# kvas7andy/unreal

Hardware: AMD Instinct MI355X
Metric: env-steps/sec (whole node), UNREAL maze 84x84 (higher is better)
Workload: dtype f32 (fp16x2-split MFMA operands, fp32 accumulate)

## Files before the change

unreal_amd/csrc/gemm_split.hip:

```cpp
#include "common.h"

namespace {

constexpr int BK = 32;
constexpr int NPL = 2;
typedef _Float16 f16x8 __attribute__((ext_vector_type(8)));
typedef _Float16 f16x2 __attribute__((ext_vector_type(2)));
constexpr int ROW_B = 80;
constexpr int FLAG_RELU = 1, FLAG_ACCUM = 2, FLAG_ATOMIC = 4, FLAG_RELU_MASK = 8, FLAG_RELU_BITS = 16;

typedef float f32x2 __attribute__((ext_vector_type(2)));
typedef unsigned int u32x2 __attribute__((ext_vector_type(2)));
typedef unsigned int u32x4 __attribute__((ext_vector_type(4)));

__device__ __forceinline__ int row_deal(int j) { return (j & ~7) | ((j & 1) << 2) | ((j >> 1) & 3); }

struct SplitArgs {
  int M, N, K;
  const float* A; int lda;
  const unsigned short* W; int ldw; long plane;
  float* C; int ldc;
  const float* bias;
  const float* mask; int ldm;
  int flags;
  int vecA;
  int nbx, nby;
  int splitk, ktiles_per_split;
  long slab_stride;
  const float* c_prev; float* c_out; float* h_out; int ld_h;
  const float* A2; int lda2, K1, K1pad;
  const float* dh_above; float* dc_io; const float* gates_act; const float* c_new; float* dpre;
  const float* a_absmax; float a_floor; const float* w_absmax; float* c_absmax0; float* c_absmax1;
};

template <int ROWS, bool VEC>
__device__ __forceinline__ f32x4 a_piece_load(const float* __restrict__ P, int ld, int rows_total, int K, int r0, int k0, int p,
                                              int tid) {
  const int id = tid + 256 * p;
  const int r = min(r0 + row_deal(id / (BK / 4)), rows_total - 1);
  const int k = k0 + (id % (BK / 4)) * 4;
  const float* row = P + (size_t)r * ld;
  if (VEC) return *reinterpret_cast<const f32x4*>(row + min(k, ld - 4));
  f32x4 v;
#pragma unroll
  for (int e = 0; e < 4; ++e) v[e] = row[min(k + e, K - 1)];
  return v;
}

__device__ __forceinline__ void split4_terms(float x0, float x1, float x2, float x3, u32x2 (&pl)[NPL]) {
  const f16x2 h01 = __builtin_convertvector((f32x2){x0, x1}, f16x2), h23 = __builtin_convertvector((f32x2){x2, x3}, f16x2);
  const f32x2 r01 = (f32x2){x0, x1} - __builtin_convertvector(h01, f32x2), r23 = (f32x2){x2, x3} - __builtin_convertvector(h23, f32x2);
  const f16x2 l01 = __builtin_convertvector(r01, f16x2), l23 = __builtin_convertvector(r23, f16x2);
  pl[0] = (u32x2){__builtin_bit_cast(unsigned int, h01), __builtin_bit_cast(unsigned int, h23)};
  pl[1] = (u32x2){__builtin_bit_cast(unsigned int, l01), __builtin_bit_cast(unsigned int, l23)};
}

template <int ROWS>
__device__ __forceinline__ void a_piece_store(unsigned char* S, f32x4 v, int klim, int p, int tid, float scale) {
  const int id = tid + 256 * p;
  const int r = row_deal(id / (BK / 4)), k = (id % (BK / 4)) * 4;
#pragma unroll
  for (int e = 0; e < 4; ++e) v[e] = k + e < klim ? v[e] * scale : 0.f;
  u32x2 pl[NPL];
  split4_terms(v[0], v[1], v[2], v[3], pl);
#pragma unroll
  for (int t = 0; t < NPL; ++t)
    *reinterpret_cast<u32x2*>(S + (t * ROWS + r) * ROW_B + k * 2) = pl[t];
}

template <int ROWS>
__device__ __forceinline__ u32x4 w_piece_load(const unsigned short* __restrict__ W, int ldw, long plane, int rows_total,
                                              int r0, int k0, int p, int tid) {
  const int id = tid + 256 * p;
  const int t = id / (ROWS * 4), r = row_deal((id / 4) % ROWS), c = id % 4;
  const int row = min(r0 + r, rows_total - 1);
  return *reinterpret_cast<const u32x4*>(W + t * plane + (size_t)row * ldw + k0 + c * 8);
}

template <int ROWS>
__device__ __forceinline__ void w_piece_store(unsigned char* S, u32x4 v, int p, int tid) {
  const int id = tid + 256 * p;
  const int t = id / (ROWS * 4), r = row_deal((id / 4) % ROWS), c = id % 4;
  *reinterpret_cast<u32x4*>(S + (t * ROWS + r) * ROW_B + c * 16) = v;
}

template <int BM, int BN, bool SWZ = false>
__device__ __forceinline__ void read_frags(const unsigned char* As, const unsigned char* Bs, int wm, int wn, int li, int kh,
                                           int ks, f16x8 (&af)[BM / 64][NPL], f16x8 (&bf)[BN / 64][NPL]) {
  const int c = 2 * ks + kh;
#pragma unroll
  for (int i = 0; i < BM / 64; ++i)
#pragma unroll
    for (int t = 0; t < NPL; ++t) {
      const int r = wm * (BM / 2) + i * 32 + li;
      af[i][t] = *reinterpret_cast<const f16x8*>(As + (t * BM + r) * ROW_B + (SWZ ? (c ^ ((r >> 4) & 3)) : c) * 16);
    }
#pragma unroll
  for (int j = 0; j < BN / 64; ++j)
#pragma unroll
    for (int t = 0; t < NPL; ++t) {
      const int r = wn * (BN / 2) + j * 32 + li;
      bf[j][t] = *reinterpret_cast<const f16x8*>(Bs + (t * BN + r) * ROW_B + (SWZ ? (c ^ ((r >> 4) & 3)) : c) * 16);
    }
}

template <int TM, int TN>
__device__ __forceinline__ void mma_frags(const f16x8 (&af)[TM][NPL], const f16x8 (&bf)[TN][NPL], f32x16 (&acc)[TM][TN]) {
#pragma unroll
  for (int i = 0; i < TM; ++i)
#pragma unroll
    for (int j = 0; j < TN; ++j) {
      f32x16 c = acc[i][j];
      c = __builtin_amdgcn_mfma_f32_32x32x16_f16(af[i][1], bf[j][0], c, 0, 0, 0);
      c = __builtin_amdgcn_mfma_f32_32x32x16_f16(af[i][0], bf[j][1], c, 0, 0, 0);
      c = __builtin_amdgcn_mfma_f32_32x32x16_f16(af[i][0], bf[j][0], c, 0, 0, 0);
      acc[i][j] = c;
    }
}

template <bool DUAL>
struct ASrc { const float* P; int ld, K, k0; };

template <bool DUAL>
__device__ __forceinline__ ASrc<DUAL> a_src(const SplitArgs& p, int kg) {
  ASrc<DUAL> s;
  if (DUAL) {
    const bool second = kg >= p.K1pad;
    s.P = second ? p.A2 : p.A; s.ld = second ? p.lda2 : p.lda;
    s.K = second ? p.K - p.K1pad : p.K1; s.k0 = second ? kg - p.K1pad : kg;
  } else {
    s.P = p.A; s.ld = p.lda; s.K = p.K; s.k0 = kg;
  }
  return s;
}

template <int BM, int BN, bool VEC, int EPI = 0, int KW = 1, bool DUAL = false>
__global__ __launch_bounds__(256 * KW, KW == 1 ? ((BM == 128 && EPI == 0) ? 3 : 2) : 1) void gemm_split_nt_kernel(SplitArgs p) {
  constexpr bool DEEP = BM == 64;
  constexpr int TM = BM / 64, TN = BN / 64;
  constexpr int PA = BM * BK / 1024, PW = NPL * BN / 64;
  constexpr int A_BYTES = NPL * BM * ROW_B, B_BYTES = NPL * BN * ROW_B;
  const float SA = pow2_scale(fmaxf(p.a_absmax ? *p.a_absmax : 0.f, p.a_floor));
  const float INV_A = pow2_inv(SA);
  const float INV_W = pow2_inv(pow2_scale(*p.w_absmax));
  constexpr bool HALF = BM == 128 && EPI == 0 && KW == 1;
  constexpr int C_BYTES = (HALF ? BM / 2 : BM) * (BN + 4) * 4;
  constexpr int OP_BYTES = A_BYTES + B_BYTES;
  constexpr int RED_BYTES = 64;
  constexpr int SMEM = OP_BYTES > (C_BYTES + RED_BYTES) ? OP_BYTES : (C_BYTES + RED_BYTES);
  static_assert(4 * KW * 4 <= RED_BYTES, "one float per wave");
  __shared__ __attribute__((aligned(16))) unsigned char smem_all[KW * SMEM];
  const int tid = KW == 1 ? (int)threadIdx.x : (int)(threadIdx.x & 255);
  const int grp = KW == 1 ? 0 : (int)(threadIdx.x >> 8);
  unsigned char* smem = smem_all + grp * SMEM;
  unsigned char* As = smem;
  unsigned char* Bs = smem + A_BYTES;

  const int L = blockIdx.x, xcd = L & 7, s = L >> 3;
  const int slab = s % p.splitk, s2 = s / p.splitk;
  const int bx = s2 % p.nbx, by = (s2 / p.nbx) * 8 + xcd;
  if (by >= p.nby) return;
  const int m0 = by * BM, n0 = bx * BN;
  if (EPI == 0) p.C += (size_t)slab * p.slab_stride;
  const int kt_base = slab * p.ktiles_per_split;
  const int nkt = min((p.K + BK - 1) / BK - kt_base, p.ktiles_per_split);
  if (nkt <= 0) return;
  const int lane = tid & 63, wave = tid >> 6;
  const int wm = wave >> 1, wn = wave & 1;
  const int li = lane & 31, kh = lane >> 5;

  f32x16 acc[TM][TN];
#pragma unroll
  for (int i = 0; i < TM; ++i)
#pragma unroll
    for (int j = 0; j < TN; ++j)
#pragma unroll
      for (int r = 0; r < 16; ++r) acc[i][j][r] = 0.f;

  f32x4 ra[2][PA];
  u32x4 rw[PW];
  const int shift = (int)((unsigned)by * 7u % (unsigned)nkt);
#define KT_AT(i) (kt_base + (((i) + shift) >= nkt ? (i) + shift - nkt : (i) + shift))
#define KG_AT(i) (KT_AT(min((i) * KW + grp, nkt - 1)) * BK)
#define KLIM(i, src) ((KW == 1 || (i) * KW + grp < nkt) ? (src).K - (src).k0 : 0)
#define A_LOAD(src, q) a_piece_load<BM, VEC>((src).P, (src).ld, p.M, (src).K, m0, (src).k0, q, tid)
  const int nit = (nkt + KW - 1) / KW;
  {
    const int k0 = KG_AT(0);
    const ASrc<DUAL> s0 = a_src<DUAL>(p, k0);
#pragma unroll
    for (int q = 0; q < PA; ++q) ra[0][q] = A_LOAD(s0, q);
#pragma unroll
    for (int q = 0; q < PW; ++q) rw[q] = w_piece_load<BN>(p.W, p.ldw, p.plane, p.N, n0, k0, q, tid);
#pragma unroll
    for (int q = 0; q < PA; ++q) a_piece_store<BM>(As, ra[0][q], KLIM(0, s0), q, tid, SA);
#pragma unroll
    for (int q = 0; q < PW; ++q) w_piece_store<BN>(Bs, rw[q], q, tid);
    const int k1 = KG_AT(1), k2 = KG_AT(2);
    const ASrc<DUAL> s1 = a_src<DUAL>(p, k1), s2_ = a_src<DUAL>(p, k2);
#pragma unroll
    for (int q = 0; q < PA; ++q) ra[0][q] = A_LOAD(s1, q);
    if (DEEP) {
#pragma unroll
      for (int q = 0; q < PA; ++q) ra[1][q] = A_LOAD(s2_, q);
    }
#pragma unroll
    for (int q = 0; q < PW; ++q) rw[q] = w_piece_load<BN>(p.W, p.ldw, p.plane, p.N, n0, k1, q, tid);
  }
  __syncthreads();

#define SPLIT_NT_TILE(S, IT)                                                                                        \
  {                                                                                                                 \
    f16x8 af[TM][NPL], bf[TN][NPL];                                                                                 \
    read_frags<BM, BN>(As, Bs, wm, wn, li, kh, 0, af, bf);                                                          \
    mma_frags<TM, TN>(af, bf, acc);                                                                                 \
    read_frags<BM, BN>(As, Bs, wm, wn, li, kh, 1, af, bf);          \
    __syncthreads();                                                               \
    const int kcur = KG_AT((IT) + 1), kw = KG_AT((IT) + 2), ka = KG_AT((IT) + (DEEP ? 3 : 2));                      \
    const ASrc<DUAL> scur = a_src<DUAL>(p, kcur), snext = a_src<DUAL>(p, ka);                                       \
    const int klim = KLIM((IT) + 1, scur);                                                                          \
    _Pragma("unroll") for (int q = 0; q < PA; ++q) {                                                                \
      a_piece_store<BM>(As, ra[S][q], klim, q, tid, SA);                                                            \
      ra[S][q] = A_LOAD(snext, q);                                                                                  \
    }                                                                                                               \
    _Pragma("unroll") for (int q = 0; q < PW; ++q) {                                                                \
      w_piece_store<BN>(Bs, rw[q], q, tid);                                                                         \
      rw[q] = w_piece_load<BN>(p.W, p.ldw, p.plane, p.N, n0, kw, q, tid);                                           \
    }                                                                                                               \
    mma_frags<TM, TN>(af, bf, acc);                                                                                 \
    __syncthreads();                                                                    \
  }
  if (DEEP) {
    for (int it = 0; it < nit; it += 2) {
      SPLIT_NT_TILE(0, it)
      if (it + 1 < nit) SPLIT_NT_TILE(1, it + 1)
    }
  } else {
    for (int it = 0; it < nit; ++it) SPLIT_NT_TILE(0, it)
  }
#undef SPLIT_NT_TILE
#undef A_LOAD
#undef KLIM
#undef KG_AT
#undef KT_AT

  if (EPI == 0 && (p.flags & FLAG_ATOMIC)) {
#pragma unroll
    for (int i = 0; i < TM; ++i)
#pragma unroll
      for (int j = 0; j < TN; ++j) {
        const int col = n0 + wn * (BN / 2) + j * 32 + li;
        if (col >= p.N) continue;
        const float bv = (p.bias && slab == 0 && grp == 0) ? p.bias[col] : 0.f;
#pragma unroll
        for (int r = 0; r < 16; ++r) {
          const int row = m0 + wm * (BM / 2) + i * 32 + (r & 3) + 8 * (r >> 2) + 4 * kh;
          const float v = (acc[i][j][r] * INV_A) * INV_W;
          if (row < p.M) atomicAdd(p.C + (size_t)row * p.ldc + col, v + bv);
        }
      }
    return;
  }
  constexpr int CLD = BN + 4;
  float* Cs = reinterpret_cast<float*>(smem);
  if (HALF) {
    const uint16_t* mbits = reinterpret_cast<const uint16_t*>(p.mask);
    const bool vecC = ((p.ldc & 3) == 0) && ((((uintptr_t)p.C) & 15) == 0) &&
                      (!p.bias || ((((uintptr_t)p.bias) & 15) == 0)) &&
                      (!(p.flags & FLAG_RELU_MASK) || (((p.ldm & 3) == 0) && ((((uintptr_t)p.mask) & 15) == 0)));
    constexpr int CV = BN / 4;
    float omax = 0.f;
#pragma unroll 1
    for (int half = 0; half < 2; ++half) {
      if (half) __syncthreads();
      if (wm == half) {
#pragma unroll
        for (int i = 0; i < TM; ++i)
#pragma unroll
          for (int j = 0; j < TN; ++j)
#pragma unroll
            for (int r = 0; r < 16; ++r)
              Cs[(i * 32 + (r & 3) + 8 * (r >> 2) + 4 * kh) * CLD + wn * (BN / 2) + j * 32 + li] =
                  (acc[i][j][r] * INV_A) * INV_W;
      }
      __syncthreads();
      for (int id = threadIdx.x; id < (BM / 2) * CV; id += 256) {
        const int r = id / CV, c4 = (id % CV) * 4;
        const int row = m0 + half * (BM / 2) + r, col = n0 + c4;
        if (row >= p.M || col >= p.N) continue;
        f32x4 v = *reinterpret_cast<const f32x4*>(Cs + r * CLD + c4);
        float* cp = p.C + (size_t)row * p.ldc + col;
        if (vecC && col + 3 < p.N) {
          if (p.bias) { const f32x4 b4 = *reinterpret_cast<const f32x4*>(p.bias + col); v += b4; }
          if (p.flags & FLAG_ACCUM) v += *reinterpret_cast<const f32x4*>(cp);
          if (p.flags & FLAG_RELU) {
#pragma unroll
            for (int e = 0; e < 4; ++e) v[e] = fmaxf(v[e], 0.f);
          }
          if (p.flags & FLAG_RELU_MASK) {
            const f32x4 m4 = *reinterpret_cast<const f32x4*>(p.mask + (size_t)row * p.ldm + col);
#pragma unroll
            for (int e = 0; e < 4; ++e) v[e] = m4[e] > 0.f ? v[e] : 0.f;
          }
          if (p.flags & FLAG_RELU_BITS) {
            const unsigned w = mbits[(size_t)row * p.ldm + (col >> 4)] >> (col & 15);
#pragma unroll
            for (int e = 0; e < 4; ++e) v[e] = ((w >> e) & 1u) ? v[e] : 0.f;
          }
          *reinterpret_cast<f32x4*>(cp) = v;
          omax = fmaxf(fmaxf(omax, fmaxf(fabsf(v[0]), fabsf(v[1]))), fmaxf(fabsf(v[2]), fabsf(v[3])));
        } else {
#pragma unroll
          for (int e = 0; e < 4; ++e) {
            if (col + e >= p.N) break;
            float x = v[e] + (p.bias ? p.bias[col + e] : 0.f);
            if (p.flags & FLAG_ACCUM) x += cp[e];
            if (p.flags & FLAG_RELU) x = fmaxf(x, 0.f);
            if (p.flags & FLAG_RELU_MASK) x = (p.mask[(size_t)row * p.ldm + col + e] > 0.f) ? x : 0.f;
            if (p.flags & FLAG_RELU_BITS) x = ((mbits[(size_t)row * p.ldm + ((col + e) >> 4)] >> ((col + e) & 15)) & 1u) ? x : 0.f;
            cp[e] = x;
            omax = fmaxf(omax, fabsf(x));
          }
        }
      }
    }
    if (p.c_absmax0) {
      __syncthreads();
      float* wmx0 = reinterpret_cast<float*>(smem_all);
      omax = wave_max(omax);
      if ((threadIdx.x & 63) == 0) wmx0[threadIdx.x >> 6] = omax;
      __syncthreads();
      if (threadIdx.x < 64) absmax_commit(p.c_absmax0, fmaxf(fmaxf(wmx0[0], wmx0[1]), fmaxf(wmx0[2], wmx0[3])));
    }
    return;
  }
#pragma unroll
  for (int i = 0; i < TM; ++i)
#pragma unroll
    for (int j = 0; j < TN; ++j)
#pragma unroll
      for (int r = 0; r < 16; ++r)
        Cs[(wm * (BM / 2) + i * 32 + (r & 3) + 8 * (r >> 2) + 4 * kh) * CLD + wn * (BN / 2) + j * 32 + li] =
            (acc[i][j][r] * INV_A) * INV_W;
  __syncthreads();
  const float* C0 = reinterpret_cast<const float*>(smem_all);
  constexpr int GSTRIDE = SMEM / 4;
  if (EPI == 1) {
    const int u0 = bx * (BN / 4);
    const bool add_pre = (p.flags & FLAG_ACCUM) != 0;
    constexpr int ITEMS = BM * (BN / 4) / (256 * KW);
    float cprev[ITEMS], pre4[ITEMS][4];
#pragma unroll
    for (int e = 0; e < ITEMS; ++e) {
      const int id = threadIdx.x + e * 256 * KW;
      const int row = min(m0 + id / (BN / 4), p.M - 1), u = u0 + id % (BN / 4);
      cprev[e] = p.c_prev[(size_t)row * 256 + u];
#pragma unroll
      for (int g4 = 0; g4 < 4; ++g4) pre4[e][g4] = add_pre ? p.C[(size_t)row * p.ldc + g4 * 256 + u] : 0.f;
    }
    static_assert((256 * KW) % (BN / 4) == 0, "a lane keeps its hidden unit over the pairs it handles");
    float bb[4];
#pragma unroll
    for (int g4 = 0; g4 < 4; ++g4) bb[g4] = p.bias[g4 * 256 + u0 + threadIdx.x % (BN / 4)];
#pragma unroll
    for (int e = 0; e < ITEMS; ++e) {
      const int id = threadIdx.x + e * 256 * KW;
      const int r = id / (BN / 4), ul = id % (BN / 4);
      const int row = m0 + r, u = u0 + ul;
      const float* cs = C0 + r * CLD + (ul >> 4) * 64 + (ul & 15);
      float s4[4];
#pragma unroll
      for (int g4 = 0; g4 < 4; ++g4) {
        float a = cs[g4 * 16];
#pragma unroll
        for (int g = 1; g < KW; ++g) a += cs[g * GSTRIDE + g4 * 16];
        s4[g4] = add_pre ? a + pre4[e][g4] : a;
      }
      const float gi = 1.f / (1.f + expf(-(s4[0] + bb[0])));
      const float gj = tanhf(s4[1] + bb[1]);
      const float gf = 1.f / (1.f + expf(-(s4[2] + bb[2] + 1.0f)));
      const float go = 1.f / (1.f + expf(-(s4[3] + bb[3])));
      const float c = cprev[e] * gf + gi * gj;
      if (row >= p.M) continue;
      float* pre = p.C + (size_t)row * p.ldc;
      pre[u] = gi; pre[256 + u] = gj; pre[512 + u] = gf; pre[768 + u] = go;
      p.c_out[(size_t)row * 256 + u] = c;
      p.h_out[(size_t)row * p.ld_h + u] = tanhf(c) * go;
    }
    return;
  }
  if (EPI == 2) {
    constexpr int ITEMS = BM * BN / (256 * KW), CH = ITEMS < 4 ? ITEMS : 4;
    float omax = 0.f;
#pragma unroll
    for (int e0 = 0; e0 < ITEMS; e0 += CH) {
      float dha[CH], dcv[CH], cn[CH], cp[CH], ga[CH][4];
#pragma unroll
      for (int e = 0; e < CH; ++e) {
        const int id = threadIdx.x + (e0 + e) * 256 * KW;
        const size_t g = (size_t)min(m0 + id / BN, p.M - 1) * 256 + n0 + id % BN;
        dha[e] = p.dh_above[g]; dcv[e] = p.dc_io[g]; cn[e] = p.c_new[g]; cp[e] = p.c_prev[g];
#pragma unroll
        for (int g4 = 0; g4 < 4; ++g4) ga[e][g4] = p.gates_act[(g / 256) * 1024 + g4 * 256 + g % 256];
      }
#pragma unroll
      for (int e = 0; e < CH; ++e) {
        const int id = threadIdx.x + (e0 + e) * 256 * KW;
        const int r = id / BN, cidx = id % BN;
        float rec = C0[r * CLD + cidx];
#pragma unroll
        for (int g = 1; g < KW; ++g) rec += C0[g * GSTRIDE + r * CLD + cidx];
        if (m0 + r >= p.M) continue;
        const size_t g = (size_t)(m0 + r) * 256 + n0 + cidx;
        const float i = ga[e][0], j = ga[e][1], f = ga[e][2], o = ga[e][3];
        const float dh = dha[e] + rec;
        const float tc = tanhf(cn[e]);
        const float dc = dcv[e] + dh * o * (1.f - tc * tc);
        float* d = p.dpre + (g / 256) * 1024 + g % 256;
        const float d0 = dc * j * i * (1.f - i), d1 = dc * i * (1.f - j * j), d2 = dc * cp[e] * f * (1.f - f),
                    d3 = dh * tc * o * (1.f - o);
        d[0] = d0; d[256] = d1; d[512] = d2; d[768] = d3;
        omax = fmaxf(fmaxf(omax, fmaxf(fabsf(d0), fabsf(d1))), fmaxf(fabsf(d2), fabsf(d3)));
        p.dc_io[g] = dc * f;
      }
    }
    {
      float* wmx = reinterpret_cast<float*>(smem_all + C_BYTES);
      omax = wave_max(omax);
      if ((threadIdx.x & 63) == 0) wmx[threadIdx.x >> 6] = omax;
      __syncthreads();
      if (threadIdx.x < 64) {
        float m = wmx[0];
#pragma unroll
        for (int g = 1; g < 4 * KW; ++g) m = fmaxf(m, wmx[g]);
        absmax_commit(p.c_absmax0, m);
        absmax_commit(p.c_absmax1, m);
      }
    }
    return;
  }
  const uint16_t* mbits = reinterpret_cast<const uint16_t*>(p.mask);
  const bool vecC = ((p.ldc & 3) == 0) && ((((uintptr_t)p.C) & 15) == 0) &&
                    (!p.bias || ((((uintptr_t)p.bias) & 15) == 0)) &&
                    (!(p.flags & FLAG_RELU_MASK) || (((p.ldm & 3) == 0) && ((((uintptr_t)p.mask) & 15) == 0)));
  constexpr int CV = BN / 4;
  float omax = 0.f;
  static_assert((BM * CV) % (256 * KW) == 0, "every lane makes the same number of passes (absmax_commit needs whole waves)");
  for (int id = threadIdx.x; id < BM * CV; id += 256 * KW) {
    const int r = id / CV, c4 = (id % CV) * 4;
    const int row = m0 + r, col = n0 + c4;
    if (row >= p.M || col >= p.N) continue;
    f32x4 v = *reinterpret_cast<const f32x4*>(C0 + r * CLD + c4);
#pragma unroll
    for (int g = 1; g < KW; ++g) v += *reinterpret_cast<const f32x4*>(C0 + g * GSTRIDE + r * CLD + c4);
    float* cp = p.C + (size_t)row * p.ldc + col;
    if (vecC && col + 3 < p.N) {
      if (p.bias) { const f32x4 b4 = *reinterpret_cast<const f32x4*>(p.bias + col); v += b4; }
      if (p.flags & FLAG_ACCUM) v += *reinterpret_cast<const f32x4*>(cp);
      if (p.flags & FLAG_RELU) {
#pragma unroll
        for (int e = 0; e < 4; ++e) v[e] = fmaxf(v[e], 0.f);
      }
      if (p.flags & FLAG_RELU_MASK) {
        const f32x4 m4 = *reinterpret_cast<const f32x4*>(p.mask + (size_t)row * p.ldm + col);
#pragma unroll
        for (int e = 0; e < 4; ++e) v[e] = m4[e] > 0.f ? v[e] : 0.f;
      }
      if (p.flags & FLAG_RELU_BITS) {
        const unsigned w = mbits[(size_t)row * p.ldm + (col >> 4)] >> (col & 15);
#pragma unroll
        for (int e = 0; e < 4; ++e) v[e] = ((w >> e) & 1u) ? v[e] : 0.f;
      }
      *reinterpret_cast<f32x4*>(cp) = v;
      omax = fmaxf(fmaxf(omax, fmaxf(fabsf(v[0]), fabsf(v[1]))), fmaxf(fabsf(v[2]), fabsf(v[3])));
    } else {
#pragma unroll
      for (int e = 0; e < 4; ++e) {
        if (col + e >= p.N) break;
        float x = v[e] + (p.bias ? p.bias[col + e] : 0.f);
        if (p.flags & FLAG_ACCUM) x += cp[e];
        if (p.flags & FLAG_RELU) x = fmaxf(x, 0.f);
        if (p.flags & FLAG_RELU_MASK) x = (p.mask[(size_t)row * p.ldm + col + e] > 0.f) ? x : 0.f;
        if (p.flags & FLAG_RELU_BITS) x = ((mbits[(size_t)row * p.ldm + ((col + e) >> 4)] >> ((col + e) & 15)) & 1u) ? x : 0.f;
        cp[e] = x;
        omax = fmaxf(omax, fabsf(x));
      }
    }
  }
  if (p.c_absmax0) {
    float* wmx0 = reinterpret_cast<float*>(smem_all + C_BYTES);
    omax = wave_max(omax);
    if ((threadIdx.x & 63) == 0) wmx0[threadIdx.x >> 6] = omax;
    __syncthreads();
    if (threadIdx.x < 64) {
      float m = wmx0[0];
#pragma unroll
      for (int g = 1; g < 4 * KW; ++g) m = fmaxf(m, wmx0[g]);
      absmax_commit(p.c_absmax0, m);
    }
  }
}

struct SplitTnArgs {
  int M, N, K;
  const float* A; int lda;
  const float* B; int ldb;
  float* C; int ldc;
  float* colsum;
  int ntx, nty, splitk, ktiles_per_split;
  const float* a_absmax; const float* b_absmax;
};

__device__ __forceinline__ int tn_m4() {
  const int t = threadIdx.x;
  return ((t >> 1) & 1) | (((t >> 4) & 1) << 1) | (((t >> 2) & 3) << 2) | (((t >> 5) & 1) << 4);
}
__device__ __forceinline__ int tn_k4() {
  const int t = threadIdx.x;
  return (t & 1) | ((t >> 6) << 1);
}

__device__ __forceinline__ void tn_piece_load(const float* __restrict__ P, int ld, int K, int c0, int k0, f32x4 (&reg)[4]) {
  const int m4 = tn_m4(), k4 = tn_k4();
  const int col = min(c0 + 4 * m4, ld - 4);
#pragma unroll
  for (int kk = 0; kk < 4; ++kk) {
    const int k = min(k0 + 4 * k4 + kk, K - 1);
    reg[kk] = *reinterpret_cast<const f32x4*>(P + (size_t)k * ld + col);
  }
}

template <int ROWS, bool RAGGED>
__device__ __forceinline__ void tn_piece_store(unsigned char* S, const f32x4 (&reg)[4], int klim, float scale) {
  const int m4 = tn_m4(), k4 = tn_k4();
  bool ok[4];
#pragma unroll
  for (int kk = 0; kk < 4; ++kk) ok[kk] = !RAGGED || 4 * k4 + kk < klim;
#pragma unroll
  for (int j = 0; j < 4; ++j) {
    const int r = 4 * m4 + j;
    u32x2 pl[NPL];
    split4_terms(ok[0] ? reg[0][j] * scale : 0.f, ok[1] ? reg[1][j] * scale : 0.f, ok[2] ? reg[2][j] * scale : 0.f,
                 ok[3] ? reg[3][j] * scale : 0.f, pl);
    const int off = (((k4 >> 1) ^ ((r >> 4) & 3)) * 2 + (k4 & 1)) * 8;
#pragma unroll
    for (int t = 0; t < NPL; ++t)
      *reinterpret_cast<u32x2*>(S + (t * ROWS + r) * ROW_B + off) = pl[t];
  }
}

template <bool RAGGED>
__device__ __forceinline__ void tn_colsum_acc(const f32x4 (&reg)[4], int klim, float w, float (&cs)[4]) {
  const int k4 = tn_k4();
#pragma unroll
  for (int kk = 0; kk < 4; ++kk) {
    const float wk = (!RAGGED || 4 * k4 + kk < klim) ? w : 0.f;
#pragma unroll
    for (int j = 0; j < 4; ++j) cs[j] = fmaf(wk, reg[kk][j], cs[j]);
  }
}

template <bool RAGGED>
__global__ __launch_bounds__(256, 2) void gemm_split_tn_kernel(SplitTnArgs p) {
  constexpr int BM = 128, BN = 128, TM = 2, TN = 2;
  constexpr int A_BYTES = NPL * BM * ROW_B, B_BYTES = NPL * BN * ROW_B;
  constexpr int OP_BYTES = A_BYTES + B_BYTES;
  __shared__ __attribute__((aligned(16))) unsigned char smem[OP_BYTES > 8 * BN * 4 ? OP_BYTES : 8 * BN * 4];
  const float SA = pow2_scale(*p.a_absmax), SB = pow2_scale(*p.b_absmax);
  const float INV_A = pow2_inv(SA), INV_B = pow2_inv(SB);
  unsigned char* As = smem;
  unsigned char* Bs = smem + A_BYTES;

  const int L = blockIdx.x, xcd = L & 7, s = L >> 3;
  const int tiles = p.ntx * p.nty;
  const int slab = (s / tiles) * 8 + xcd, tile = s % tiles;
  if (slab >= p.splitk) return;
  const int bx = tile % p.ntx, by = tile / p.ntx;
  const int m0 = by * BM, n0 = bx * BN;
  const int nk_total = (p.K + BK - 1) / BK;
  const int kt0 = slab * p.ktiles_per_split, kt1 = min(nk_total, kt0 + p.ktiles_per_split);
  if (kt0 >= kt1) return;
  const int nkt = kt1 - kt0;
  const int lane = threadIdx.x & 63, wave = threadIdx.x >> 6;
  const int wm = wave >> 1, wn = wave & 1;
  const int li = lane & 31, kh = lane >> 5;

  f32x16 acc[TM][TN];
#pragma unroll
  for (int i = 0; i < TM; ++i)
#pragma unroll
    for (int j = 0; j < TN; ++j)
#pragma unroll
      for (int r = 0; r < 16; ++r) acc[i][j][r] = 0.f;

  constexpr int TN_FLUSH = 8;
  f32x16 tot[TM][TN];
#pragma unroll
  for (int i = 0; i < TM; ++i)
#pragma unroll
    for (int j = 0; j < TN; ++j)
#pragma unroll
      for (int r = 0; r < 16; ++r) tot[i][j][r] = 0.f;
  f32x4 ra[4], rb[4];
  const float csw = (p.colsum != nullptr && by == 0) ? 1.f : 0.f;
  float cs[4] = {0.f, 0.f, 0.f, 0.f};
  tn_piece_load(p.A, p.lda, p.K, m0, kt0 * BK, ra);
  tn_piece_load(p.B, p.ldb, p.K, n0, kt0 * BK, rb);
  tn_piece_store<BM, RAGGED>(As, ra, p.K - kt0 * BK, SA);
  tn_piece_store<BN, RAGGED>(Bs, rb, p.K - kt0 * BK, SB);
  tn_colsum_acc<RAGGED>(rb, p.K - kt0 * BK, csw, cs);
  {
    const int k1 = (kt0 + min(1, nkt - 1)) * BK;
    tn_piece_load(p.A, p.lda, p.K, m0, k1, ra);
    tn_piece_load(p.B, p.ldb, p.K, n0, k1, rb);
  }
  __syncthreads();

  for (int it = 0; it < nkt; ++it) {
    f16x8 af[TM][NPL], bf[TN][NPL];
    read_frags<BM, BN, true>(As, Bs, wm, wn, li, kh, 0, af, bf);
    mma_frags<TM, TN>(af, bf, acc);
    read_frags<BM, BN, true>(As, Bs, wm, wn, li, kh, 1, af, bf);
    __syncthreads();
    const int kcur = (kt0 + min(it + 1, nkt - 1)) * BK, knext = (kt0 + min(it + 2, nkt - 1)) * BK;
    tn_piece_store<BM, RAGGED>(As, ra, p.K - kcur, SA);
    tn_piece_load(p.A, p.lda, p.K, m0, knext, ra);
    tn_piece_store<BN, RAGGED>(Bs, rb, p.K - kcur, SB);
    tn_colsum_acc<RAGGED>(rb, p.K - kcur, (it + 1 < nkt) ? csw : 0.f, cs);
    tn_piece_load(p.B, p.ldb, p.K, n0, knext, rb);
    mma_frags<TM, TN>(af, bf, acc);
    if ((it + 1) % TN_FLUSH == 0) {
#pragma unroll
      for (int i = 0; i < TM; ++i)
#pragma unroll
        for (int j = 0; j < TN; ++j)
#pragma unroll
          for (int r = 0; r < 16; ++r) { tot[i][j][r] += acc[i][j][r]; acc[i][j][r] = 0.f; }
    }
    __syncthreads();
  }
#pragma unroll
  for (int i = 0; i < TM; ++i)
#pragma unroll
    for (int j = 0; j < TN; ++j)
#pragma unroll
      for (int r = 0; r < 16; ++r) acc[i][j][r] += tot[i][j][r];

  if (csw != 0.f) {
    float* red = reinterpret_cast<float*>(smem);
    const int m4 = tn_m4(), k4 = tn_k4();
#pragma unroll
    for (int j = 0; j < 4; ++j) red[k4 * BN + 4 * m4 + j] = cs[j];
    __syncthreads();
    if (threadIdx.x < BN && n0 + threadIdx.x < p.N) {
      float v = 0.f;
#pragma unroll
      for (int k = 0; k < 8; ++k) v += red[k * BN + threadIdx.x];
      atomicAdd(p.colsum + n0 + threadIdx.x, v);
    }
  }
#pragma unroll
  for (int i = 0; i < TM; ++i)
#pragma unroll
    for (int j = 0; j < TN; ++j) {
      const int col = n0 + wn * (BN / 2) + j * 32 + li;
      if (col >= p.N) continue;
#pragma unroll
      for (int r = 0; r < 16; ++r) {
        const int row = m0 + wm * (BM / 2) + i * 32 + (r & 3) + 8 * (r >> 2) + 4 * kh;
        if (row < p.M) atomicAdd(p.C + (size_t)row * p.ldc + col, (acc[i][j][r] * INV_A) * INV_B);
      }
    }
}

__global__ __launch_bounds__(256) void split_planes_f16x2_kernel(int rows, int cols, const float* __restrict__ src, int ld_src,
                                                                 int transpose, unsigned short* __restrict__ dst, int ld_dst,
                                                                 long plane, int row_perm, const float* __restrict__ w_absmax) {
  __shared__ float t[32][33];
  const float sw = pow2_scale(*w_absmax);
  const int c0 = blockIdx.x * 32, r0 = blockIdx.y * 32;
  const int tx = threadIdx.x & 31, ty = threadIdx.x >> 5;
  for (int y = ty; y < 32; y += 8)
    if (r0 + y < rows && c0 + tx < cols) t[y][tx] = src[(size_t)(r0 + y) * ld_src + c0 + tx];
  __syncthreads();
  for (int y = ty; y < 32; y += 8) {
    int orow = transpose ? c0 + y : r0 + y;
    const int ocol = transpose ? r0 + tx : c0 + tx;
    if (row_perm == 1) orow = ((orow & 255) >> 4) * 64 + (orow >> 8) * 16 + (orow & 15);
    const bool ok = transpose ? (c0 + y < cols && r0 + tx < rows) : (r0 + y < rows && c0 + tx < cols);
    if (!ok) continue;
    const float x = (transpose ? t[tx][y] : t[y][tx]) * sw;
    const _Float16 h = (_Float16)x;
    const _Float16 l = (_Float16)(x - (float)h);
    dst[(size_t)orow * ld_dst + ocol] = __builtin_bit_cast(unsigned short, h);
    dst[plane + (size_t)orow * ld_dst + ocol] = __builtin_bit_cast(unsigned short, l);
  }
}

__global__ __launch_bounds__(256) void absmax_kernel(int rows, int cols, const float* __restrict__ x, int ld, float* slot) {
  float m = 0.f;
  if (ld == cols && (cols & 3) == 0 && ((((uintptr_t)x) & 15) == 0)) {
    const long n4 = (long)rows * cols / 4;
    const f32x4* x4 = reinterpret_cast<const f32x4*>(x);
    for (long i = (long)blockIdx.x * 256 + threadIdx.x; i < n4; i += (long)gridDim.x * 256) {
      const f32x4 v = x4[i];
      m = fmaxf(fmaxf(m, fmaxf(fabsf(v[0]), fabsf(v[1]))), fmaxf(fabsf(v[2]), fabsf(v[3])));
    }
  } else {
    const int wave = (blockIdx.x * 256 + threadIdx.x) >> 6, nw = (gridDim.x * 256) >> 6, lane = threadIdx.x & 63;
    for (int r = wave; r < rows; r += nw)
      for (int c = lane; c < cols; c += 64) m = fmaxf(m, fabsf(x[(size_t)r * ld + c]));
  }
  __shared__ float wm[4];
  m = wave_max(m);
  if ((threadIdx.x & 63) == 0) wm[threadIdx.x >> 6] = m;
  __syncthreads();
  if (threadIdx.x < 64) absmax_commit(slot, fmaxf(fmaxf(wm[0], wm[1]), fmaxf(wm[2], wm[3])));
}

struct MultiAbsDesc { const float* src; float* wmax; long n; long block0; };
struct MultiSplitDesc { const float* src; unsigned short* dst; const float* wmax; long rows, cols, ld_src, transpose, row_perm, ld_dst, plane, tiles_x, block0; };

__global__ __launch_bounds__(256) void multi_absmax_kernel(const MultiAbsDesc* __restrict__ descs, int n_desc) {
// ... 338 lines not shown
```

Before: 3.715 million.

## Peel final K iterations and prefetch LSTM epilogue inputs during last MMA

Peels the last one to two K-loop iterations of the split-fp16 GEMM so the final tiles skip redundant global loads. The global loads for the LSTM forward and backward epilogues (c_prev, previous pre-activations, bias, dh, dc, gate activations) are issued during the last tile's MMA instead of after the loop. This is meant to hide epilogue load latency behind compute. In exchange it raises register pressure, adds complex per-group trip-count logic with extra barrier matching, and pins the FMA contraction in the backward gate math by hand.

```diff
diff --git a/unreal_amd/csrc/gemm_split.hip b/unreal_amd/csrc/gemm_split.hip
--- a/unreal_amd/csrc/gemm_split.hip
+++ b/unreal_amd/csrc/gemm_split.hip
@@ -209,6 +209,39 @@
   }
   __syncthreads();
 
+  constexpr int E1_ITEMS = BM * (BN / 4) / (256 * KW);
+  constexpr int E2_ITEMS = BM * BN / (256 * KW), E2_CH = E2_ITEMS < 4 ? E2_ITEMS : 4;
+  float e1_cprev[E1_ITEMS], e1_pre[E1_ITEMS][4], e1_bias[4];
+  constexpr int E2_PF = E2_CH < 3 ? E2_CH : 3;
+  float e2_in[E2_PF][8];
+  auto epi_prefetch = [&]() __attribute__((always_inline)) {
+    if (EPI == 1) {
+      const int u0 = bx * (BN / 4);
+      const bool add_pre = !DUAL && (p.flags & FLAG_ACCUM) != 0;
+#pragma unroll
+      for (int e = 0; e < E1_ITEMS; ++e) {
+        const int id = threadIdx.x + e * 256 * KW;
+        const int row = min(m0 + id / (BN / 4), p.M - 1), u = u0 + id % (BN / 4);
+        e1_cprev[e] = p.c_prev[(size_t)row * 256 + u];
+#pragma unroll
+        for (int g4 = 0; g4 < 4; ++g4) e1_pre[e][g4] = add_pre ? p.C[(size_t)row * p.ldc + g4 * 256 + u] : 0.f;
+      }
+#pragma unroll
+      for (int g4 = 0; g4 < 4; ++g4) e1_bias[g4] = p.bias[g4 * 256 + u0 + threadIdx.x % (BN / 4)];
+    }
+    if (EPI == 2) {
+#pragma unroll
+      for (int e = 0; e < E2_PF; ++e) {
+        const int id = threadIdx.x + e * 256 * KW;
+        const size_t g = (size_t)min(m0 + id / BN, p.M - 1) * 256 + n0 + id % BN;
+        e2_in[e][0] = p.dh_above[g]; e2_in[e][1] = p.dc_io[g]; e2_in[e][2] = p.c_new[g]; e2_in[e][3] = p.c_prev[g];
+#pragma unroll
+        for (int g4 = 0; g4 < 4; ++g4) e2_in[e][4 + g4] = p.gates_act[(g / 256) * 1024 + g4 * 256 + g % 256];
+      }
+    }
+  };
+  constexpr bool PEEL = !(BM == 128 && EPI == 0);
+
 #define SPLIT_NT_TILE(S, IT)                                                                                        \
   {                                                                                                                 \
     f16x8 af[TM][NPL], bf[TN][NPL];                                                                                 \
@@ -230,14 +263,64 @@
     mma_frags<TM, TN>(af, bf, acc);                                                                                 \
     __syncthreads();                                                                    \
   }
-  if (DEEP) {
-    for (int it = 0; it < nit; it += 2) {
-      SPLIT_NT_TILE(0, it)
-      if (it + 1 < nit) SPLIT_NT_TILE(1, it + 1)
-    }
+#define SPLIT_NT_TAIL(IT, LOAD_W, MID)                                                                              \
+  {                                                                                                                 \
+    f16x8 af[TM][NPL], bf[TN][NPL];                                                                                 \
+    read_frags<BM, BN>(As, Bs, wm, wn, li, kh, 0, af, bf);                                                          \
+    mma_frags<TM, TN>(af, bf, acc);                                                                                 \
+    read_frags<BM, BN>(As, Bs, wm, wn, li, kh, 1, af, bf);                                                          \
+    __syncthreads();                                                                                                \
+    const int kcur = KG_AT((IT) + 1), kw = KG_AT((IT) + 2);                                                         \
+    const ASrc<DUAL> scur = a_src<DUAL>(p, kcur);                                                                   \
+    const int klim = KLIM((IT) + 1, scur);                                                                          \
+    const bool odd = DEEP && (((IT) & 1) != 0);                                                                     \
+    _Pragma("unroll") for (int q = 0; q < PA; ++q) {                                                                \
+      const f32x4 v0 = ra[0][q], v1 = DEEP ? ra[1][q] : v0;                                                         \
+      a_piece_store<BM>(As, odd ? v1 : v0, klim, q, tid, SA);                                                       \
+    }                                                                                                               \
+    _Pragma("unroll") for (int q = 0; q < PW; ++q) {                                                                \
+      w_piece_store<BN>(Bs, rw[q], q, tid);                                                                         \
+      if (LOAD_W) rw[q] = w_piece_load<BN>(p.W, p.ldw, p.plane, p.N, n0, kw, q, tid);                               \
+    }                                                                                                               \
+    MID                                                                                                             \
+    mma_frags<TM, TN>(af, bf, acc);                                                                                 \
+    __syncthreads();                                                                                                \
+  }
+  if (PEEL) {
+    const int nit_g = KW == 1 ? nit : max((nkt - grp + KW - 1) / KW, 1);
+    const int nmain = nit_g - (DEEP ? 3 : 2);
+    if (DEEP) {
+      for (int it = 0; it < nmain; it += 2) {
+        SPLIT_NT_TILE(0, it)
+        if (it + 1 < nmain) SPLIT_NT_TILE(1, it + 1)
+      }
+      if (nit_g >= 3) SPLIT_NT_TAIL(nit_g - 3, true, )
+    } else {
+      for (int it = 0; it < nmain; ++it) SPLIT_NT_TILE(0, it)
+    }
+    if (nit_g >= 2) SPLIT_NT_TAIL(nit_g - 2, false, epi_prefetch();)
+    else epi_prefetch();
+    {
+      f16x8 af[TM][NPL], bf[TN][NPL];
+      read_frags<BM, BN>(As, Bs, wm, wn, li, kh, 0, af, bf);
+      mma_frags<TM, TN>(af, bf, acc);
+      read_frags<BM, BN>(As, Bs, wm, wn, li, kh, 1, af, bf);
+      mma_frags<TM, TN>(af, bf, acc);
+      __syncthreads();
+    }
+    if (KW > 1 && nit_g < nit) { __syncthreads(); __syncthreads(); }
   } else {
-    for (int it = 0; it < nit; ++it) SPLIT_NT_TILE(0, it)
-  }
+    if (DEEP) {
+      for (int it = 0; it < nit; it += 2) {
+        SPLIT_NT_TILE(0, it)
+        if (it + 1 < nit) SPLIT_NT_TILE(1, it + 1)
+      }
+    } else {
+      for (int it = 0; it < nit; ++it) SPLIT_NT_TILE(0, it)
+    }
+    epi_prefetch();
+  }
+#undef SPLIT_NT_TAIL
 #undef SPLIT_NT_TILE
 #undef A_LOAD
 #undef KLIM
@@ -349,19 +432,11 @@
     const int u0 = bx * (BN / 4);
     const bool add_pre = (p.flags & FLAG_ACCUM) != 0;
     constexpr int ITEMS = BM * (BN / 4) / (256 * KW);
-    float cprev[ITEMS], pre4[ITEMS][4];
-#pragma unroll
-    for (int e = 0; e < ITEMS; ++e) {
-      const int id = threadIdx.x + e * 256 * KW;
-      const int row = min(m0 + id / (BN / 4), p.M - 1), u = u0 + id % (BN / 4);
-      cprev[e] = p.c_prev[(size_t)row * 256 + u];
-#pragma unroll
-      for (int g4 = 0; g4 < 4; ++g4) pre4[e][g4] = add_pre ? p.C[(size_t)row * p.ldc + g4 * 256 + u] : 0.f;
-    }
+    static_assert(ITEMS == E1_ITEMS, "epi_prefetch covers every pair");
     static_assert((256 * KW) % (BN / 4) == 0, "a lane keeps its hidden unit over the pairs it handles");
-    float bb[4];
-#pragma unroll
-    for (int g4 = 0; g4 < 4; ++g4) bb[g4] = p.bias[g4 * 256 + u0 + threadIdx.x % (BN / 4)];
+    const float (&cprev)[ITEMS] = e1_cprev;
+    const float (&pre4)[ITEMS][4] = e1_pre;
+    const float (&bb)[4] = e1_bias;
 #pragma unroll
     for (int e = 0; e < ITEMS; ++e) {
       const int id = threadIdx.x + e * 256 * KW;
@@ -390,13 +465,19 @@
     return;
   }
   if (EPI == 2) {
-    constexpr int ITEMS = BM * BN / (256 * KW), CH = ITEMS < 4 ? ITEMS : 4;
+    constexpr int ITEMS = E2_ITEMS, CH = E2_CH;
     float omax = 0.f;
 #pragma unroll
     for (int e0 = 0; e0 < ITEMS; e0 += CH) {
       float dha[CH], dcv[CH], cn[CH], cp[CH], ga[CH][4];
 #pragma unroll
       for (int e = 0; e < CH; ++e) {
+        if (e0 == 0 && e < E2_PF) {
+          dha[e] = e2_in[e][0]; dcv[e] = e2_in[e][1]; cn[e] = e2_in[e][2]; cp[e] = e2_in[e][3];
+#pragma unroll
+          for (int g4 = 0; g4 < 4; ++g4) ga[e][g4] = e2_in[e][4 + g4];
+          continue;
+        }
         const int id = threadIdx.x + (e0 + e) * 256 * KW;
         const size_t g = (size_t)min(m0 + id / BN, p.M - 1) * 256 + n0 + id % BN;
         dha[e] = p.dh_above[g]; dcv[e] = p.dc_io[g]; cn[e] = p.c_new[g]; cp[e] = p.c_prev[g];
@@ -415,10 +496,15 @@
         const float i = ga[e][0], j = ga[e][1], f = ga[e][2], o = ga[e][3];
         const float dh = dha[e] + rec;
         const float tc = tanhf(cn[e]);
-        const float dc = dcv[e] + dh * o * (1.f - tc * tc);
+        float dc, d0, d1, d2, d3;
+        {
+#pragma clang fp contract(off)
+          const float tt = tc * tc;
+          dc = __builtin_fmaf(dh * o, 1.f - tt, dcv[e]);
+          d0 = dc * j * i * (1.f - i); d1 = dc * i * __builtin_fmaf(-j, j, 1.f); d2 = dc * cp[e] * f * (1.f - f);
+          d3 = dh * tc * o * (1.f - o);
+        }
         float* d = p.dpre + (g / 256) * 1024 + g % 256;
-        const float d0 = dc * j * i * (1.f - i), d1 = dc * i * (1.f - j * j), d2 = dc * cp[e] * f * (1.f - f),
-                    d3 = dh * tc * o * (1.f - o);
         d[0] = d0; d[256] = d1; d[512] = d2; d[768] = d3;
         omax = fmaxf(fmaxf(omax, fmaxf(fabsf(d0), fabsf(d1))), fmaxf(fabsf(d2), fabsf(d3)));
         p.dc_io[g] = dc * f;
```

Measured after the change: 3.736 million, median of 5. About the same (+0.6%).
